# forestagostinelli/DeepCubeA

Hardware: AMD Instinct MI355X
Metric: A* nodes expanded/sec on cube3, batch 20k (higher is better)
Workload: dtype u8 states / f64 cost keys / f32 heuristic

## Files before the change

### deepcubea_amd/csrc/dca_engine.hip

```cpp
#include <string.h>

#include <new>
#include <vector>

#include "dca_common.h"
#include "dca_tile.h"

namespace dca {

constexpr int NBIN = 4096;
constexpr int kBinsPerThread = NBIN / 1024;
constexpr int kLgNbin = 12;
constexpr int kSub = 2048;
constexpr int kScanBlocks = 256;
constexpr int kCollectBlocks = 512;
constexpr int kRankBlocks = 256;
constexpr uint32_t kTinyBin = 512;
constexpr int kSortCap = 8192;
constexpr int RT = 512;
constexpr int kRegEnt = 16;
constexpr uint32_t kLdsEnt = RT * kRegEnt;
constexpr int kStash = 2560;
constexpr int kSegs = NBIN + 1 + kSub;
constexpr uint32_t kGiantBin = 8192;
// ... 119 lines not shown
    uint32_t* coop_off;
    uint64_t* part;
    uint64_t* tmp_key;
    uint32_t* tmp_id;
    uint16_t* tmp_f;
    uint32_t* tmp_idx;
    uint64_t* ord_key;
    uint32_t* ord_id;
    uint32_t* big_list;
    uint64_t* pop_key;
    uint32_t *pop_id, *pop_g;
    uint32_t *child_slot, *child_next, *child_v0;
    uint8_t *child_flags, *child_multi;
    float* child_h;
    uint8_t* nnet_in;
    uint8_t* onehot;
    uint8_t* root_nnet;
    int32_t* d_moves;
    Ctl* ctl;
    unsigned long long* prof;
    uint32_t* kept_pos;
    uint32_t* pk_n;
    uint32_t* pk_src;
    uint8_t* pk_nnet;
    uint8_t* pk_onehot;
    const float* pk_h;
    uint32_t pk_stride, inst;
    int pk_dtype;
};

__device__ __forceinline__ const IterState& st_cur(const Ctl* c) { return c->S[c->iters & 1]; }
__device__ __forceinline__ const IterState& st_next(const Ctl* c) { return c->S[(c->iters + 1) & 1]; }

__device__ __forceinline__ void fresh_binning(const Ctl* c, uint32_t buf, uint64_t& kmin, uint32_t& shift) {
    kmin = c->rng[buf].kmin;
    uint64_t kmax = c->rng[buf].kmax;
    const uint64_t T = c->T;
    if (T != ~0ull && T > kmax) kmax = T;
    shift = kmax > kmin ? select_shift(kmin, kmax) : 0u;
}

struct Stamp {
    unsigned long long* p;
    unsigned long long t0;
    __device__ __forceinline__ Stamp(const Eng& E, int kid) : p(nullptr), t0(0) {
        if (E.prof != nullptr && threadIdx.x == 0) {
            p = E.prof + ((size_t)kid * kProfSlots + (blockIdx.x & (kProfSlots - 1))) * 2;
            t0 = wall_clock64();
        }
    }
    __device__ __forceinline__ ~Stamp() {
        if (p) {
            atomicMin(p, t0);
            atomicMax(p + 1, (unsigned long long)wall_clock64());
        }
    }
};

__device__ __forceinline__ void prof_begin(const Eng& E, int kid) {
    if (E.prof != nullptr && threadIdx.x == 0)
        atomicMin(E.prof + ((size_t)kid * kProfSlots + (blockIdx.x & (kProfSlots - 1))) * 2, (unsigned long long)wall_clock64());
}
__device__ __forceinline__ void prof_end(const Eng& E, int kid) {
    if (E.prof != nullptr && threadIdx.x == 0)
        atomicMax(E.prof + ((size_t)kid * kProfSlots + (blockIdx.x & (kProfSlots - 1))) * 2 + 1, (unsigned long long)wall_clock64());
}

__device__ __forceinline__ void open_append(const Eng& E, Ctl* c, uint32_t buf, bool pred, uint64_t key, uint32_t id) {
    unsigned long long mask = __ballot(pred);
    if (mask == 0) return;
    int lane = threadIdx.x & 63;
    int leader = __ffsll((long long)mask) - 1;
    uint32_t cnt = (uint32_t)__popcll(mask);
    uint32_t basep = 0;
    uint64_t kmn = pred ? key : ~0ull, kmx = pred ? key : 0ull;
    for (int o = 32; o > 0; o >>= 1) {
        uint64_t a = __shfl_xor(kmn, o), b = __shfl_xor(kmx, o);
        kmn = a < kmn ? a : kmn;
        kmx = b > kmx ? b : kmx;
    }
    if (lane == leader) {
        basep = atomicAdd(&c->open_n[buf].v, cnt);
        atomicMin((unsigned long long*)&c->rng[buf].kmin, (unsigned long long)kmn);
        atomicMax((unsigned long long*)&c->rng[buf].kmax, (unsigned long long)kmx);
    }
    basep = __shfl(basep, leader);
    if (pred) {
        uint32_t pos = basep + (uint32_t)__popcll(mask & ((1ull << lane) - 1ull));
        if (pos < (buf < 2 ? E.front_cap : E.max_nodes)) {
            E.open_key[buf][pos] = key;
            E.open_id[buf][pos] = id;
        } else {
            c->failed = 1;
        }
    }
}
// ... 1022 lines not shown
                    const uint32_t p = atomicAdd(&L.st_n, 1u);
                    keys[idx] = DEAD;
                    if (p < (uint32_t)kStashG) {
                        st_key[p] = k[i];
                        st_idx[p] = idx;
                        st_f[p] = (uint16_t)f;
                        if (atomicAdd(&lcnt[f], 1u) == 0u) nzf[atomicAdd(&L.nz_n, 1u)] = (uint16_t)f;
                    } else {
                        const uint32_t pos = seg_base(f) + atomicAdd(&E.fill[f], 1u);
                        if (pos < seg_end(f)) {
                            E.tmp_key[pos] = k[i];
                            E.tmp_id[pos] = id[i];
                            E.tmp_f[pos] = (uint16_t)f;
                            E.tmp_idx[pos] = idx;
                        } else {
                            c->failed = 1;
                        }
                    }
                }
            }
            __syncthreads();
            if (L.st_n + TILE_D > (uint32_t)kStashG) flush();
        }
    }
    __syncthreads();
    flush();
    return BAR_PASS;
}

template <bool FUSED>
__global__ __launch_bounds__(256) void k_sel_collect(const Eng* __restrict__ engs) {
    const Eng& E = engs[blockIdx.y];
    Ctl* c = E.ctl;
    if (c->done) return;
    Stamp stamp(E, P_SEL_COLLECT);
    extern __shared__ __attribute__((aligned(16))) uint8_t collect_lds[];
    CollectLds& L = *reinterpret_cast<CollectLds*>(collect_lds);
    const uint32_t t = threadIdx.x;
    SelParams P;
    {
        const uint32_t b = c->cur_f, on0 = c->open_n[0].v, on1 = c->open_n[1].v;
        P.b = b;
        P.n = b ? on1 : on0;
        P.kmin = c->sel_kmin;
        P.shift = c->shift;
        P.want = c->want;
    }
    if constexpr (FUSED) {
        constexpr int PER = NBIN / 256;
        const uint32_t lane = t & 63, wv = t >> 6;
        uint32_t v[PER], sum = 0;
        {
            const uint4* h4 = reinterpret_cast<const uint4*>(E.hist + PER * t);
#pragma unroll
            for (int q = 0; q < PER / 4; q++) {
                const uint4 x = h4[q];
                v[4 * q] = x.x;
                v[4 * q + 1] = x.y;
                v[4 * q + 2] = x.z;
                v[4 * q + 3] = x.w;
            }
#pragma unroll
            for (int k = 0; k < PER; k++) sum += v[k];
        }
        uint32_t incl = sum;
        for (int o = 1; o < 64; o <<= 1) {
            const uint32_t u = __shfl_up(incl, o);
            if (lane >= (uint32_t)o) incl += u;
        }
        if (lane == 63) L.wsum[wv] = incl;
        if (t == 0) L.bstar = 0;
        __syncthreads();
        uint32_t run = incl - sum;
        for (uint32_t w = 0; w < wv; w++) run += L.wsum[w];
        const uint32_t want = P.want;
#pragma unroll
        for (int k = 0; k < PER; k++) {
            L.pre[PER * t + k] = run;
            if (run < want && want <= run + v[k]) L.bstar = PER * t + k;
            run += v[k];
        }
        if (t == 255) L.pre[NBIN] = run;
        __syncthreads();
        if (want == 0) {
            if (blockIdx.x == 0 && t == 0) {
                c->failed = 1;
                c->done = 1;
            }
            return;
// ... 134 lines not shown
                const uint32_t f = bin_of(k[i], kmin, shift);
                const uint32_t p = atomicAdd(&L.st_n, 1u);
                keys[idx] = DEAD;
                if (p < kStash) {
                    st_key[p] = k[i];
                    st_idx[p] = idx;
                    st_f[p] = (uint16_t)f;
                    if (atomicAdd(&L.lcnt[f], 1u) == 0u) nzf[atomicAdd(&L.nz_n, 1u)] = (uint16_t)f;
                } else {
                    const uint32_t pos = L.pre[f] + atomicAdd(&E.fill[f], 1u);
                    if (pos < L.pre[f + 1]) {
                        E.tmp_key[pos] = k[i];
                        E.tmp_id[pos] = ids[idx];
                        E.tmp_f[pos] = (uint16_t)f;
                        E.tmp_idx[pos] = idx;
                    } else {
                        c->failed = 1;
                    }
                }
            }
        }
        __syncthreads();
        if (L.st_n + TILE > (uint32_t)kStash) flush();
    }
    __syncthreads();
    flush();
}


constexpr int kRankStack = 512;
constexpr uint32_t kDirectMax = 512;
constexpr uint32_t kSubMax = 512;

struct RankItem {
    uint32_t off, n, need, src;
    uint32_t g, G;
    uint32_t nopush;
};
struct RankShared {
    uint32_t cnt[kSub + 64];
    uint32_t off[kSub + 1];
    uint32_t wsum[16];
    uint64_t red_lo[32], red_hi[32];
    uint64_t vmin_hi, vmin_lo;
    uint64_t kmin, kspan;
    uint32_t imin, ispan;
    uint32_t bits, tsub, sp, fail;
    uint32_t ret_base, ret_cnt;
    RankItem stack[kRankStack];
};

__device__ __forceinline__ void emit_pop(const Eng& E, Ctl* c, uint32_t rank, uint64_t key, uint32_t id) {
    E.pop_key[rank] = key;
    E.pop_id[rank] = id;
    if (id & ID_SOLVED) {
        if (E.sem == DCA_SEM_PY)
            atomicMin(&c->goal_best, ((unsigned long long)(uint32_t)E.g[id & ID_MASK] << 32) | rank);
        else
            atomicMin(&c->first_solved, rank);
    }
}
__device__ __forceinline__ void emit_ranked(const Eng& E, Ctl* c, uint32_t nf, bool live, uint32_t rank, uint32_t want,
                                            uint64_t key, uint32_t id) {
    if (live && rank < want) emit_pop(E, c, rank, key, id);
    const bool back = live && rank >= want;
    const unsigned long long mask = __ballot(back);
    if (mask == 0) return;
    const int lane = threadIdx.x & 63;
    const int leader = __ffsll((long long)mask) - 1;
    uint32_t basep = 0;
    if (lane == leader) basep = atomicAdd(&c->ret_n.v, (uint32_t)__popcll(mask));
    basep = __shfl(basep, leader);
    if (back) {
        const uint32_t slot = E.tmp_idx[basep + (uint32_t)__popcll(mask & ((1ull << lane) - 1ull))];
        E.open_key[nf][slot] = key;
        E.open_id[nf][slot] = id;
    }
}
__device__ __forceinline__ void ret_begin(Ctl* c, RankShared& S, uint32_t nf, uint32_t count) {
    __syncthreads();
    if (threadIdx.x == 0) {
        S.ret_base = count ? atomicAdd(&c->ret_n.v, count) : 0u;
        S.ret_cnt = 0;
    }
    __syncthreads();
}
struct RetAcc {};
__device__ __forceinline__ void ret_put(const Eng& E, Ctl* c, RankShared& S, uint32_t nf, bool pred, uint64_t key,
                                        uint32_t id, RetAcc& acc) {
    const unsigned long long mask = __ballot(pred);
    if (mask == 0) return;
    const int lane = threadIdx.x & 63;
    const int leader = __ffsll((long long)mask) - 1;
    uint32_t basep = 0;
    if (lane == leader) basep = atomicAdd(&S.ret_cnt, (uint32_t)__popcll(mask));
    basep = __shfl(basep, leader);
    if (pred) {
        const uint32_t slot = E.tmp_idx[S.ret_base + basep + (uint32_t)__popcll(mask & ((1ull << lane) - 1ull))];
        E.open_key[nf][slot] = key;
        E.open_id[nf][slot] = id;
    }
}
__device__ __forceinline__ void ret_end(Ctl* c, uint32_t nf, RetAcc acc) {}
template <int NJ>
__device__ __forceinline__ void ret_put_many(const Eng& E, RankShared& S, uint32_t nf, uint32_t n_ord, uint32_t preds,
                                             const uint64_t* key, const uint32_t* id) {
    const uint32_t cnt = (uint32_t)__popc(preds);
    const int lane = threadIdx.x & 63;
    uint32_t incl = cnt;
    for (int o = 1; o < 64; o <<= 1) {
        const uint32_t u = __shfl_up(incl, o);
        if (lane >= o) incl += u;
    }
    const uint32_t total = __shfl(incl, 63);
    if (total == 0) return;
    uint32_t basep = 0;
    if (lane == 63) basep = atomicAdd(&S.ret_cnt, total);
    basep = __shfl(basep, 63);
    uint32_t r = S.ret_base + basep + incl - cnt;
    uint32_t slot[NJ];
#pragma unroll
    for (int j = 0; j < NJ; j++) {
        slot[j] = E.tmp_idx[r < n_ord ? r : n_ord - 1];
        r += (preds >> j) & 1u;
    }
#pragma unroll
    for (int j = 0; j < NJ; j++)
        if ((preds >> j) & 1u) {
            E.open_key[nf][slot[j]] = key[j];
            E.open_id[nf][slot[j]] = id[j];
        }
}

__device__ __forceinline__ void rank_small_entries(const Eng& E, Ctl* c, RankShared& S, uint64_t* LK, uint32_t* LI,
                                                   uint32_t nf, uint32_t p0, uint32_t n_ord, uint32_t want) {
    const uint32_t t = threadIdx.x;
    const uint32_t plast = (p0 + RT - 1 < n_ord ? p0 + RT - 1 : n_ord - 1);
    const uint32_t f_lo = E.tmp_f[p0], f_hi = E.tmp_f[plast];
    const uint32_t lo = E.pre[f_lo], hi = E.pre[f_hi + 1];
    const bool staged = hi - lo <= kLdsEnt && f_hi - f_lo + 2 <= (uint32_t)kSub;
    if (staged) {
        for (uint32_t i = t; i < hi - lo; i += RT) {
            LK[i] = E.tmp_key[lo + i];
            LI[i] = E.tmp_id[lo + i];
        }
        for (uint32_t i = t; i < f_hi - f_lo + 2; i += RT) S.off[i] = E.pre[f_lo + i];
    }
    __syncthreads();
    const uint32_t p = p0 + t;
    bool live = p < n_ord;
    uint64_t k = 0;
    uint32_t id = 0, rank = 0;
    if (live) {
        const uint32_t f = E.tmp_f[p];
        const uint32_t o = staged ? S.off[f - f_lo] : E.pre[f], e = staged ? S.off[f - f_lo + 1] : E.pre[f + 1];
        if (e - o > kTinyBin) {
            live = false;
        } else if (staged) {
            k = LK[p - lo];
            id = LI[p - lo];
            rank = o;
            for (uint32_t j = o - lo; j < e - lo; j++) rank += pair_less(LK[j], LI[j], k, id) ? 1u : 0u;
        } else {
            k = E.tmp_key[p];
            id = E.tmp_id[p];
            rank = o;
            for (uint32_t j = o; j < e; j++) rank += pair_less(E.tmp_key[j], E.tmp_id[j], k, id) ? 1u : 0u;
        }
    }
    emit_ranked(E, c, nf, live, rank, want, k, id);
    __syncthreads();
// ... 88 lines not shown
    if (lane == 63) S.wsum[wv] = incl;
    __syncthreads();
    uint32_t run = incl - s4;
    for (uint32_t w = 0; w < wv; w++) run += S.wsum[w];
#pragma unroll
    for (int k = 0; k < PER; k++) {
        const uint32_t i = PER * t + k;
        if (i < nsub) {
            S.off[i] = run;
            S.cnt[i] = 0;
            if (run < need && need <= run + v[k]) S.tsub = i;
            if (i + 1 == nsub) S.off[nsub] = run + v[k];
        }
        run += v[k];
    }
    __syncthreads();
}

__device__ __forceinline__ void rank_push(RankShared& S, const RankItem& it, uint32_t tsub, uint32_t need, bool refinable,
                                          uint32_t lo = 0u, uint32_t hi = ~0u) {
    for (uint32_t sb = lo + threadIdx.x; sb <= tsub && sb < hi; sb += RT) {
        const uint32_t s0 = S.off[sb], e0 = S.off[sb + 1];
        if (e0 - s0 > kSubMax && refinable) {
            const uint32_t slot = atomicAdd(&S.sp, 1u);
            if (slot < (uint32_t)kRankStack)
                S.stack[slot] = RankItem{it.off + s0, e0 - s0, sb == tsub ? need - s0 : e0 - s0, it.src ^ 1u, 0u, 1u,
                                         (it.G > 1u || it.nopush) ? 1u : 0u};
            else
                S.fail = 1;
        }
    }
}

__device__ __noinline__ void rank_item(const Eng& E, Ctl* c, RankShared& S, uint64_t* LK, uint32_t* LI, uint32_t nf,
                                       uint32_t want, RankItem it) {
    const uint32_t t = threadIdx.x;
    const uint64_t* __restrict__ K = (it.src ? E.ord_key : E.tmp_key) + it.off;
    const uint32_t* __restrict__ I = (it.src ? E.ord_id : E.tmp_id) + it.off;
    uint64_t* __restrict__ K2 = (it.src ? E.tmp_key : E.ord_key) + it.off;
    uint32_t* __restrict__ I2 = (it.src ? E.tmp_id : E.ord_id) + it.off;
    const uint32_t n = it.n, need = it.need;
    if (n <= kDirectMax) {
        if (t < n) {
            LK[t] = K[t];
            LI[t] = I[t];
        }
        __syncthreads();
        ret_begin(c, S, nf, n - need);
        RetAcc acc{};
        const bool live = t < n;
        uint64_t k = 0;
        uint32_t id = 0, rank = 0;
        if (live) {
            k = LK[t];
            id = LI[t];
            for (uint32_t j = 0; j < n; j++) rank += pair_less(LK[j], LI[j], k, id) ? 1u : 0u;
            if (rank < need) emit_pop(E, c, it.off + rank, k, id);
        }
        ret_put(E, c, S, nf, live && rank >= need, k, id, acc);
        ret_end(c, nf, acc);
        __syncthreads();
        return;
    }
    uint32_t lg = 0;
    while ((8u << lg) <= n && lg < 11) lg++;
    if (lg < 11) lg++;
    if (n <= kLdsEnt) {
        uint64_t ek[kRegEnt];
// ... 18 lines not shown
            }
            rank_range64(S, kmn, kmx, imn, imx);
        }
        prof_end(E, P_RB_LOAD);
        prof_begin(E, P_RB_COUNT);
        const bool idmode = S.kspan == 0;
        const uint64_t kbase = S.kmin, span = idmode ? (uint64_t)S.ispan : S.kspan;
        const uint32_t ibase = S.imin;
        const uint32_t bits = span ? (uint32_t)(64 - __clzll((long long)span)) : 0u;
        if (lg > bits) lg = bits;
        const uint32_t nsub = 1u << lg, shc = bits - lg;
        const bool refinable = (shc > 0 || !idmode) && !it.nopush;
        const uint32_t lo_sub = (uint32_t)((uint64_t)nsub * it.g / it.G), hi_sub = (uint32_t)((uint64_t)nsub * (it.g + 1u) / it.G);
#pragma unroll
        for (int j = 0; j < kRegEnt; j++) {
            ek[j] = idmode ? (uint64_t)((ei[j] & ID_MASK) - ibase) : ek[j] - kbase;
            if (t + (uint32_t)RT * j < n) atomicAdd(&S.cnt[(uint32_t)(ek[j] >> shc)], 1u);
        }
        __syncthreads();
        rank_prefix(S, nsub, need);
        prof_end(E, P_RB_COUNT);
        prof_begin(E, P_RB_SCATTER);
        if (E.prof != nullptr) {
            uint32_t mx = 0;
            for (uint32_t sb = t; sb < nsub; sb += RT) mx = max(mx, S.off[sb + 1] - S.off[sb]);
            if (mx > 16) atomicMax(&c->dbg_maxsub, mx);
        }
        const uint32_t tsub = S.tsub;
        const bool tsub_pushed = S.off[tsub + 1] - S.off[tsub] > kSubMax && refinable;
        const uint32_t in_hi = hi_sub < tsub + 1u ? hi_sub : tsub + 1u;
        const uint32_t ret_lo = lo_sub > tsub + 1u ? lo_sub : tsub + 1u;
        ret_begin(c, S, nf, (ret_lo < hi_sub ? S.off[hi_sub] - S.off[ret_lo] : 0u) +
                                ((tsub >= lo_sub && tsub < hi_sub && !tsub_pushed) ? S.off[tsub + 1] - need : 0u));
        const uint32_t n_ord = c->n_ord;
        {
            uint32_t inm = 0, retm = 0, pos[kRegEnt];
#pragma unroll
            for (int j = 0; j < kRegEnt; j++) {
                const uint32_t sub = (uint32_t)(ek[j] >> shc);
                const bool live = t + (uint32_t)RT * j < n, in = live && sub >= lo_sub && sub < in_hi;
                inm |= (in ? 1u : 0u) << j;
                retm |= (live && sub >= ret_lo && sub < hi_sub ? 1u : 0u) << j;
                pos[j] = S.off[in ? sub : 0u] + atomicAdd(&S.cnt[in ? sub : (uint32_t)kSub + (t & 63u)], in ? 1u : 0u);
            }
#pragma unroll
            for (int j = 0; j < kRegEnt; j++) {
                if ((inm >> j) & 1u) {
                    LK[pos[j]] = ek[j];
                    LI[pos[j]] = ei[j];
                }
                ek[j] = idmode ? kbase : kbase + ek[j];
            }
            ret_put_many<kRegEnt>(E, S, nf, n_ord, retm, ek, ei);
        }
        __syncthreads();
        prof_end(E, P_RB_SCATTER);
        prof_begin(E, P_RB_ORDER);
        const uint32_t p_lo = S.off[lo_sub], p_hi = in_hi > lo_sub ? S.off[in_hi] : p_lo;
        constexpr int U = 4;
        for (uint32_t p0 = p_lo; p0 < p_hi; p0 += RT * U) {
            uint64_t o[U];
            uint32_t id[U], s0[U], cn[U], rank[U], livem = 0, bigm = 0, trip = 0;
#pragma unroll
            for (int u = 0; u < U; u++) {
                const uint32_t p = p0 + (uint32_t)u * RT + t;
                livem |= (p < p_hi ? 1u : 0u) << u;
                o[u] = LK[p < p_hi ? p : p_hi - 1];
// ... 54 lines not shown
#pragma unroll
            for (int j = 0; j < kRegEnt; j++)
                if (b0 + t + (uint32_t)RT * j < n) {
                    const u128 v = comp_of(ek[j], ei[j]);
                    vmin = v < vmin ? v : vmin;
                    vmax = v > vmax ? v : vmax;
                }
        }
        rank_range(S, vmin, vmax);
    }
    const u128 base = ((u128)S.vmin_hi << 64) | S.vmin_lo;
    const uint32_t bits = S.bits;
    if (lg > bits) lg = bits;
    const uint32_t nsub = 1u << lg, shc = bits - lg;
    for (uint32_t b0 = 0; b0 < n; b0 += kLdsEnt) {
        uint64_t ek[kRegEnt];
        uint32_t ei[kRegEnt];
#pragma unroll
        for (int j = 0; j < kRegEnt; j++) {
            const uint32_t i = b0 + t + (uint32_t)RT * j, ic = i < n ? i : n - 1;
            ek[j] = K[ic];
            ei[j] = I[ic];
        }
#pragma unroll
        for (int j = 0; j < kRegEnt; j++)
            if (b0 + t + (uint32_t)RT * j < n) atomicAdd(&S.cnt[sub_of(ek[j], ei[j], base, shc, nsub)], 1u);
    }
    __syncthreads();
    rank_prefix(S, nsub, need);
    const uint32_t tsub = S.tsub;
    const bool tsub_pushed = S.off[tsub + 1] - S.off[tsub] > kSubMax && shc > 0;
    ret_begin(c, S, nf, (n - S.off[tsub + 1]) + (tsub_pushed ? 0u : S.off[tsub + 1] - need));
    RetAcc acc{};
    const uint32_t n_ord_all = c->n_ord;
    for (uint32_t b0 = 0; b0 < n; b0 += kLdsEnt) {
        uint64_t ek[kRegEnt];
        uint32_t ei[kRegEnt];
#pragma unroll
        for (int j = 0; j < kRegEnt; j++) {
            const uint32_t i = b0 + t + (uint32_t)RT * j, ic = i < n ? i : n - 1;
            ek[j] = K[ic];
            ei[j] = I[ic];
        }
        uint32_t retm = 0;
#pragma unroll
        for (int j = 0; j < kRegEnt; j++) {
            const bool live = b0 + t + (uint32_t)RT * j < n;
            uint32_t sub = 0;
            if (live) {
                sub = sub_of(ek[j], ei[j], base, shc, nsub);
                if (sub <= tsub) {
                    const uint32_t p = S.off[sub] + atomicAdd(&S.cnt[sub], 1u);
                    K2[p] = ek[j];
                    I2[p] = ei[j];
                }
            }
            retm |= (live && sub > tsub ? 1u : 0u) << j;
        }
        ret_put_many<kRegEnt>(E, S, nf, n_ord_all, retm, ek, ei);
    }
    __syncthreads();
    const uint32_t m = S.off[tsub + 1];
    for (uint32_t p0 = 0; p0 < m; p0 += RT) {
        const uint32_t p = p0 + t;
        bool live = p < m;
        uint64_t k = 0;
        uint32_t id = 0, rank = 0;
        if (live) {
            k = K2[p];
            id = I2[p];
            const uint32_t sub = sub_of(k, id, base, shc, nsub);
            const uint32_t s0 = S.off[sub], e0 = S.off[sub + 1];
            if (e0 - s0 > kSubMax && shc > 0) {
                live = false;
            } else {
                rank = s0;
                for (uint32_t j = s0; j < e0; j++) rank += pair_less(K2[j], I2[j], k, id) ? 1u : 0u;
                if (rank < need) emit_pop(E, c, it.off + rank, k, id);
            }
        }
        ret_put(E, c, S, nf, live && rank >= need, k, id, acc);
    }
    rank_push(S, it, tsub, need, shc > 0);
    ret_end(c, nf, acc);
    __syncthreads();
}

__global__ __launch_bounds__(RT) void k_rank(const Eng* __restrict__ engs) {
    const Eng& E = engs[blockIdx.y];
    Ctl* c = E.ctl;
    if (c->done) return;
    Stamp stamp(E, P_RANK);
    __shared__ RankShared S;
    extern __shared__ __attribute__((aligned(16))) uint8_t rank_lds[];
    uint64_t* LK = reinterpret_cast<uint64_t*>(rank_lds);
    uint32_t* LI = reinterpret_cast<uint32_t*>(rank_lds + (size_t)kLdsEnt * 8);
    const uint32_t t = threadIdx.x;
    const uint32_t nf = c->cur_f;
    const uint32_t tseg = c->tseg, want = c->want;
    const uint32_t n_big = c->n_big, n_ord = c->n_ord;
    if (blockIdx.x == gridDim.x - 1) {
        const uint32_t bstar = c->bstar, pre_b = c->pre_b, cn_star = c->cn_star;
        if (want != 0) {
            for (uint32_t bin = t; bin < bstar; bin += RT) E.hist[bin] = 0;
            if (t == 0) E.hist[bstar] = cn_star - (want - pre_b);
        }
        for (uint32_t i = t; i < (uint32_t)kSegs; i += RT) E.fill[i] = 0;
        if (c->giant)
            for (uint32_t i = t; i < (uint32_t)(kMaxLevels * kSub); i += RT) E.subhist[i] = 0;
    }
    {
        Stamp sub(E, P_RANK_SMALL);
        for (uint32_t p0 = blockIdx.x * RT; p0 < n_ord; p0 += gridDim.x * RT)
            rank_small_entries(E, c, S, LK, LI, nf, p0, n_ord, want);
    }
    Stamp sub2(E, P_RANK_BIG);
    for (uint32_t bi = (blockIdx.x + gridDim.x - 64u) % gridDim.x; bi < n_big; bi += gridDim.x) {
        const uint32_t unit = E.big_list[bi];
        const uint32_t f = unit & 0xFFFFu;
        const uint32_t o = E.pre[f], n = E.pre[f + 1] - o;
        __syncthreads();
        if (t == 0) {
            S.stack[0] = RankItem{o, n, (f == tseg) ? want - o : n, 0u, (unit >> 16) & 15u, unit >> 20, 0u};
            S.sp = 1;
            S.fail = 0;
        }
        for (;;) {
            __syncthreads();
            const uint32_t sp = S.sp;
            if (sp == 0 || sp > (uint32_t)kRankStack) break;
            const RankItem it = S.stack[sp - 1];
            __syncthreads();
            if (t == 0) S.sp = sp - 1;
            __syncthreads();
            rank_item(E, c, S, LK, LI, nf, want, it);
        }
        if (t == 0 && (S.fail || S.sp != 0)) c->failed = 1;
    }
}

__device__ __forceinline__ void close_pop(const Eng& E, Ctl* c, const IterState& S0, uint32_t it, uint32_t want,
                                          uint32_t npop, uint32_t base, bool fail) {
    IterState N = S0;
    if (E.sem == DCA_SEM_PY) {
        const unsigned long long gb = c->goal_best;
        if (gb != ~0ull) {
            c->stop_after = 1;
            c->goal_id = E.pop_id[(uint32_t)(gb & 0xFFFFFFFFull)] & ID_MASK;
        }
    } else {
        const uint32_t fs = c->first_solved;
        if (fs != NIL) {
            const float cst = (float)cost_of_key(E.pop_key[fs]);
            if (E.B == 1) {
                N.best_id = E.pop_id[fs] & ID_MASK;
                N.best_cost = cst;
                N.has_best = 1;
                c->stop_after = 1;
            } else if (!S0.has_best || S0.best_cost > cst) {
                N.best_id = E.pop_id[fs] & ID_MASK;
                N.best_cost = cst;
                N.has_best = 1;
            }
        }
        if (S0.has_best && (float)cost_of_key(E.pop_key[0]) >= N.best_cost) c->stop_after = 1;
    }
    if (fail) {
        c->failed = 1;
        c->done = 1;
        c->front_dead.v -= want;
        return;
    }
    const uint32_t m = npop * (uint32_t)E.A;
    N.npop = npop;
    N.m = m;
    N.base = base;
    N.pool_n = base + m;
    c->S[(it + 1) & 1] = N;
    c->gen += (int64_t)m;
    c->expanded += npop;
}

constexpr uint8_t F_KEEP = 1, F_MIN = 2, F_NEW = 4;

// ... 20 lines not shown
            }
        }
    } else {
        uint32_t z = 0xFFFFu;
#pragma unroll
        for (int b = 3; b >= 0; b--)
            if (4 * w + b < (uint32_t)EV::D && ((pw >> (8 * b)) & 0xFFu) == 0u) z = 4 * w + b;
        for (int o = 8; o > 0; o >>= 1) {
            const uint32_t y = (uint32_t)__shfl_xor((int)z, o);
            z = y < z ? y : z;
        }
        z = z < (uint32_t)EV::D ? z : 0u;
        const uint32_t sw = (uint32_t)npuzzle_swap(DIM, (int)z, (int)a);
#pragma unroll
        for (uint32_t b = 0; b < 4; b++) {
            const uint32_t i = 4 * w + b;
            const uint32_t src = i < (uint32_t)EV::D ? ((i == z) ? sw : i) : 0u;
            const uint32_t v = (uint32_t)__shfl((int)pw, gbase + (int)(src >> 2));
            if (i < (uint32_t)EV::D) out |= ((i == sw) ? 0u : ((v >> (8 * (src & 3))) & 0xFFu)) << (8 * b);
        }
    }
    return out;
}

constexpr int kEngTile = 16;
template <int ENV, int DIM, int OH>
__global__ __launch_bounds__(kThreads) void k_expand(const Eng* __restrict__ engs, int heur_id, int write_nn) {
    const Eng& E = engs[blockIdx.y];
    using EV = EnvT<ENV, DIM>;
    using TL = Tile<ENV, DIM, kEngTile>;
    constexpr int kTileParents = kEngTile;
    constexpr int TP = kEngTile;
    Ctl* c = E.ctl;
    if (c->done) return;
    Stamp stamp(E, P_EXPAND);
    extern __shared__ __attribute__((aligned(16))) uint8_t smem[];
    uint8_t* lpar = smem;
    uint8_t* ltab = smem + TL::PAR_BYTES;
    uint8_t* lst = smem + TL::LDS_BYTES;
    __shared__ uint32_t l_pid[TP], l_g[TP];
    __shared__ uint32_t l_qn, l_qcc[kThreads], l_qrep[kThreads], l_qres[kThreads];
    __shared__ uint32_t l_ohq;
    static_assert((EV::D + 3) / 4 < 16, "no spare lane per row for the parent's path cost");
    const uint32_t it = (uint32_t)c->iters;
    const IterState S0 = c->S[it & 1];
    const uint32_t want = c->want;
    uint32_t npop = want;
    if (E.sem == DCA_SEM_CPP) {
        const uint32_t fs = c->first_solved;
        if (fs != NIL) npop = fs + 1;
    }
    const uint32_t base = (S0.pool_n + 15u) & ~15u;
    const bool fail = (uint64_t)base + (uint64_t)npop * (uint64_t)EV::A > (uint64_t)E.max_nodes;
    const uint32_t cur_new = c->cur_f;
    if (blockIdx.x == 0 && threadIdx.x == 0) close_pop(E, c, S0, it, want, npop, base, fail);
    if (fail) return;
    const uint32_t r0 = blockIdx.x * kTileParents;
    if (E.sem == DCA_SEM_CPP && r0 + kTileParents > npop) {
        uint32_t r = r0 + threadIdx.x;
        bool back = threadIdx.x < kTileParents && r >= npop && r < want;
        open_append(E, c, cur_new, back, back ? E.pop_key[r] : 0, back ? E.pop_id[r] : 0);
        if (back) atomicAdd(&E.hist[bin_of(E.pop_key[r], c->sel_kmin, c->shift)], 1u);
    }
    if (r0 >= npop) return;
    const uint32_t np = min((uint32_t)kTileParents, npop - r0);
    if (OH != 0 && threadIdx.x == 0) l_ohq = 0;
    {
        constexpr int WPR = (EV::D + 3) / 4;
        static_assert(WPR <= 16, "row wider than 64 bytes");
        const uint32_t w = threadIdx.x & 15;
#pragma unroll
        for (uint32_t r = threadIdx.x >> 4; r < (uint32_t)TP; r += 16) {
        if (r < np && w == WPR) {
            const uint32_t pid = E.pop_id[r0 + r] & ID_MASK;
            l_pid[r] = pid;
            l_g[r] = (uint32_t)E.g[pid];
        }
        if (r < np && w < WPR) {
            const uint8_t* row = E.state + (size_t)(E.pop_id[r0 + r] & ID_MASK) * EV::D;
            uint32_t v = 0;
            if (4 * w + 4 <= EV::D) {
                __builtin_memcpy(&v, row + 4 * w, 4);
            } else {
                for (int b = 0; 4 * w + b < EV::D; b++) v |= (uint32_t)row[4 * w + b] << (8 * b);
            }
#pragma unroll
            for (int b = 0; b < 4; b++)
                if (4 * w + b < EV::D) lpar[r * EV::D + 4 * w + b] = (uint8_t)(v >> (8 * b));
        }
        }
    }
    if constexpr (ENV == DCA_ENV_CUBE3) stage_tables<ENV, DIM>(ltab, lpar, np);
    __syncthreads();
    if constexpr (ENV != DCA_ENV_CUBE3) {
        stage_tables<ENV, DIM>(ltab, lpar, np);
        __syncthreads();
    }
    TL t{lpar, ltab};
    const uint32_t nchild = np * EV::A;
    const uint32_t j0 = r0 * EV::A;

    auto oh_emit = [&]() {
        if constexpr (OH != 0) {
            constexpr uint32_t ROW = EV::D * EV::DEPTH;
            constexpr uint32_t EPC = 16 / OH;
            const uint32_t te = nchild * ROW;
            const uint32_t one16 = E.oh_dtype == DCA_DT_F16 ? 0x3C00u : 0x3F80u;
            uint8_t* goh = E.onehot + (size_t)j0 * ROW * OH;
            const uint32_t nch = (te + EPC - 1) / EPC;
            auto staged_nnet = [&](uint32_t i) -> uint32_t {
                const uint32_t b = lst[i];
                return ENV == DCA_ENV_CUBE3 ? (b * 57u) >> 9 : b;
// ... 396 lines not shown
}

__device__ __forceinline__ void commit_ticket(const Eng& E, Ctl* c) {
    __syncthreads();
    if (threadIdx.x == 0) {
        uint32_t t = atomicAdd(&c->ticket_a.v, 1u);
        if (t == gridDim.x - 1) {
            c->ticket_a.v = 0;
            c->iters += 1;
            if (c->stop_after || c->failed) {
                c->done = 1;
            } else {
                const uint32_t fb = c->cur_f;
                const uint32_t live = __hip_atomic_load(&c->open_n[fb].v, __ATOMIC_RELAXED, __HIP_MEMORY_SCOPE_AGENT) -
                                      __hip_atomic_load(&c->front_dead.v, __ATOMIC_RELAXED, __HIP_MEMORY_SCOPE_AGENT) - c->front_above;
                c->want = live < (uint32_t)E.B ? live : (uint32_t)E.B;
                c->ret_n.v = 0;
                c->goal_best = ~0ull;
                c->first_solved = NIL;
                c->gbar.v = 0;
                c->grange.kmin = ~0ull;
                c->grange.kmax = 0;
                c->grange.imin = ~0u;
                c->grange.imax = 0;
            }
        }
    }
}

template <bool FUSED>
__global__ __launch_bounds__(1024) void k_commit(const Eng* __restrict__ engs, int packed) {
    const Eng& E = engs[blockIdx.y];
    Ctl* c = E.ctl;
    if (c->done) return;
    Stamp stamp(E, P_COMMIT);
    __shared__ uint32_t sh[3 * 16 + 3];
    __shared__ uint32_t lh[NBIN];
    __shared__ uint64_t red[4][16];
    const IterState& S1 = st_next(c);
    const uint32_t m = S1.m, base = S1.base;
    const uint32_t fb = c->cur_f, bb = c->cur_b;
    const uint64_t T = c->T;
    const uint32_t j = blockIdx.x * 1024 + threadIdx.x;
    if (blockIdx.x * 1024 >= m) {
        commit_ticket(E, c);
        return;
    }
    uint64_t rng_snap;
    {
        const uint32_t sl = threadIdx.x < 4 ? threadIdx.x : 0u;
        const uint32_t sbuf = sl < 2 ? fb : bb;
        const uint64_t* sp = (sl & 1) ? &c->rng[sbuf].kmax : &c->rng[sbuf].kmin;
        asm volatile("global_load_dwordx2 %0, %1, off" : "=v"(rng_snap) : "v"(sp) : "memory");
    }
    for (int k = 0; k < kBinsPerThread; k++) lh[kBinsPerThread * threadIdx.x + k] = 0;
    const uint64_t bin_kmin = c->sel_kmin;
    const uint32_t bin_shift = c->shift;
    __syncthreads();
    const bool live = j < m;
    const uint32_t id = base + j;
    bool keep = false, is_new = false;
    uint32_t gj = 0, my_slot = 0;
    float h_early = 0.f;
    uint8_t solved_early = 0;
    if (live) {
        if (!packed) h_early = E.child_h[j];
        solved_early = E.solved[id];
        const uint8_t fl = E.child_flags[j];
        is_new = (fl & F_NEW) != 0;
        gj = E.pop_g[j / (uint32_t)E.A] + 1u;
        const uint32_t slot = E.child_slot[j];
        my_slot = slot;
        bool is_min;
        uint32_t first = j;
        bool multi = false;
        if constexpr (FUSED) {
            multi = E.child_multi[j] != 0;
            const Dec d = decide_child(E, base, m, j, slot, E.child_v0[j], gj, multi);
            keep = d.keep;
            is_min = d.is_min;
            first = d.first;
        } else {
            keep = (fl & F_KEEP) != 0;
            is_min = (fl & F_MIN) != 0;
        }
        if (keep && is_min) {
            E.tab[slot].g = gj;
            if (E.sem == DCA_SEM_CPP) {
                uint32_t rep = (uint32_t)E.tab[slot].entry;
                if (FUSED && rep >= base) rep = base + first;
                if (rep != id) {
                    E.g[rep] = (int32_t)gj;
                    E.parent[rep] = E.parent[id];
                    E.move[rep] = E.move[id];
                }
            }
        }
        if (FUSED && multi && j == first) fix_representative(E, base, slot, id);
        E.child_multi[j] = 0;
    }
    uint64_t key = 0;
    uint32_t pid_flag = 0;
    if (keep) {
        const float hraw = packed ? E.pk_h[E.kept_pos[j]] : h_early;
        const float hv = fmaxf(hraw, 0.0f);
        const bool ns = solved_early == 0;
        pid_flag = ns ? 0u : ID_SOLVED;
        double cost;
        if (E.sem == DCA_SEM_PY) {
            cost = __dadd_rn(__dmul_rn(E.w, (double)gj), __dmul_rn((double)hv, ns ? 1.0 : 0.0));
        } else {
            cost = (double)__fadd_rn(__fmul_rn(hv, ns ? 1.0f : 0.0f), __fmul_rn(E.wf, (float)gj));
        }
        key = key_of_cost(cost);
    }
    const bool tof = keep && key <= T, tob = keep && key > T;
    const uint32_t hbin = c->hbin;
    if (tof) {
        const uint32_t f = bin_of(key, bin_kmin, bin_shift);
        if (f < hbin) atomicAdd(&lh[f], 1u);
    }
    const uint32_t cnt[3] = {tof ? 1u : 0u, tob ? 1u : 0u, is_new ? 1u : 0u};
    uint32_t* const ctr[3] = {&c->open_n[fb].v, &c->open_n[bb].v, &c->closed_n.v};
    uint32_t pos[3];
    block_reserveK<1024, 3>(cnt, ctr, pos, sh);
    static_assert(kBinsPerThread % 2 == 0, "bins are flushed in aligned pairs");
    if (kBinsPerThread * threadIdx.x < hbin) {
#pragma unroll
        for (int k = 0; k < kBinsPerThread; k += 2) {
            const uint32_t v0 = lh[kBinsPerThread * threadIdx.x + k], v1 = lh[kBinsPerThread * threadIdx.x + k + 1];
            if (v0 | v1)
                atomicAdd(reinterpret_cast<unsigned long long*>(&E.hist[kBinsPerThread * threadIdx.x + k]),
                          (unsigned long long)v0 | ((unsigned long long)v1 << 32));
        }
    }
    if (is_new && pos[2] < E.max_nodes) E.closed_slots[pos[2]] = my_slot;
    if (tof) {
        if (pos[0] < E.front_cap) {
            E.open_key[fb][pos[0]] = key;
            E.open_id[fb][pos[0]] = id | pid_flag;
        } else {
            c->failed = 1;
        }
    } else if (tob) {
        if (pos[1] < E.max_nodes) {
            E.open_key[bb][pos[1]] = key;
            E.open_id[bb][pos[1]] = id | pid_flag;
        } else {
            c->failed = 1;
        }
// ... 1019 lines not shown
```

Before: 94.75 million.

## Hoist control and input loads to kernel heads across collect, rank, expand, commit

Across several kernels, the control-block fields, histogram slices, per-child inputs and per-parent pop ids are now loaded in one batch at kernel entry, before the done check. Empty asm statements force these loads to be issued early so their latencies overlap instead of being serialised behind dependent branches. The rank kernel also gets a compact RankEng struct whose pointers are pinned to scalar registers through a constant-address-space load and readfirstlane. The cost is speculative loads, using clamped indices, on blocks that would otherwise exit early, plus higher register pressure.

Result: no change. 95.18 million, median of 4 (+0.5%).

```diff
diff --git a/deepcubea_amd/csrc/dca_engine.hip b/deepcubea_amd/csrc/dca_engine.hip
--- a/deepcubea_amd/csrc/dca_engine.hip
+++ b/deepcubea_amd/csrc/dca_engine.hip
@@ -175,6 +175,19 @@
 __device__ __forceinline__ const IterState& st_cur(const Ctl* c) { return c->S[c->iters & 1]; }
 __device__ __forceinline__ const IterState& st_next(const Ctl* c) { return c->S[(c->iters + 1) & 1]; }
 
+using GCtl = const __attribute__((address_space(1))) Ctl*;
+__device__ __forceinline__ GCtl global_ctl(const Ctl* c) { return (GCtl)c; }
+__device__ __forceinline__ IterState load_state(GCtl c, int k) {
+    IterState s;
+    s.pool_n = c->S[k].pool_n;
+    s.npop = c->S[k].npop;
+    s.m = c->S[k].m;
+    s.base = c->S[k].base;
+    s.best_id = c->S[k].best_id;
+    s.has_best = c->S[k].has_best;
+    s.best_cost = c->S[k].best_cost;
+    return s;
+}
 __device__ __forceinline__ void fresh_binning(const Ctl* c, uint32_t buf, uint64_t& kmin, uint32_t& shift) {
     kmin = c->rng[buf].kmin;
     uint64_t kmax = c->rng[buf].kmax;
@@ -186,7 +199,8 @@
 struct Stamp {
     unsigned long long* p;
     unsigned long long t0;
-    __device__ __forceinline__ Stamp(const Eng& E, int kid) : p(nullptr), t0(0) {
+    template <class EngT>
+    __device__ __forceinline__ Stamp(const EngT& E, int kid) : p(nullptr), t0(0) {
         if (E.prof != nullptr && threadIdx.x == 0) {
             p = E.prof + ((size_t)kid * kProfSlots + (blockIdx.x & (kProfSlots - 1))) * 2;
             t0 = wall_clock64();
@@ -200,11 +214,13 @@
     }
 };
 
-__device__ __forceinline__ void prof_begin(const Eng& E, int kid) {
+template <class EngT>
+__device__ __forceinline__ void prof_begin(const EngT& E, int kid) {
     if (E.prof != nullptr && threadIdx.x == 0)
         atomicMin(E.prof + ((size_t)kid * kProfSlots + (blockIdx.x & (kProfSlots - 1))) * 2, (unsigned long long)wall_clock64());
 }
-__device__ __forceinline__ void prof_end(const Eng& E, int kid) {
+template <class EngT>
+__device__ __forceinline__ void prof_end(const EngT& E, int kid) {
     if (E.prof != nullptr && threadIdx.x == 0)
         atomicMax(E.prof + ((size_t)kid * kProfSlots + (blockIdx.x & (kProfSlots - 1))) * 2 + 1, (unsigned long long)wall_clock64());
 }
@@ -1293,29 +1309,42 @@
 __global__ __launch_bounds__(256) void k_sel_collect(const Eng* __restrict__ engs) {
     const Eng& E = engs[blockIdx.y];
     Ctl* c = E.ctl;
-    if (c->done) return;
+    const GCtl gc = global_ctl(c);
+    const uint32_t t = threadIdx.x;
+    constexpr int PER = NBIN / 256;
+    const int32_t done = gc->done;
+    const uint32_t hb = gc->cur_f, on0 = gc->open_n[0].v, on1 = gc->open_n[1].v;
+    const uint64_t hkmin = gc->sel_kmin;
+    const uint32_t hshift = gc->shift, hwant = gc->want;
+    typedef uint32_t u32x4 __attribute__((ext_vector_type(4)));
+    u32x4 hx[PER / 4] = {};
+    if constexpr (FUSED) {
+        const u32x4* h4 = reinterpret_cast<const u32x4*>(E.hist + PER * t);
+#pragma unroll
+        for (int q = 0; q < PER / 4; q++) hx[q] = h4[q];
+        asm volatile("" ::"v"(done), "v"(hb), "v"(on0), "v"(on1), "v"(hkmin), "v"(hshift), "v"(hwant), "v"(hx[0]), "v"(hx[1]),
+                     "v"(hx[2]), "v"(hx[3]));
+    } else {
+        asm volatile("" ::"v"(done), "v"(hb), "v"(on0), "v"(on1), "v"(hkmin), "v"(hshift), "v"(hwant));
+    }
+    if (done) return;
     Stamp stamp(E, P_SEL_COLLECT);
     extern __shared__ __attribute__((aligned(16))) uint8_t collect_lds[];
     CollectLds& L = *reinterpret_cast<CollectLds*>(collect_lds);
-    const uint32_t t = threadIdx.x;
     SelParams P;
-    {
-        const uint32_t b = c->cur_f, on0 = c->open_n[0].v, on1 = c->open_n[1].v;
-        P.b = b;
-        P.n = b ? on1 : on0;
-        P.kmin = c->sel_kmin;
-        P.shift = c->shift;
-        P.want = c->want;
-    }
+    P.b = hb;
+    P.n = hb ? on1 : on0;
+    P.kmin = hkmin;
+    P.shift = hshift;
+    P.want = hwant;
     if constexpr (FUSED) {
-        constexpr int PER = NBIN / 256;
+        static_assert(PER == 16, "the head requests four 16-byte pieces of the histogram per thread");
         const uint32_t lane = t & 63, wv = t >> 6;
         uint32_t v[PER], sum = 0;
         {
-            const uint4* h4 = reinterpret_cast<const uint4*>(E.hist + PER * t);
 #pragma unroll
             for (int q = 0; q < PER / 4; q++) {
-                const uint4 x = h4[q];
+                const u32x4 x = hx[q];
                 v[4 * q] = x.x;
                 v[4 * q + 1] = x.y;
                 v[4 * q + 2] = x.z;
@@ -1516,6 +1545,59 @@
 constexpr uint32_t kDirectMax = 512;
 constexpr uint32_t kSubMax = 512;
 
+using CEng = const __attribute__((address_space(4))) Eng*;
+struct RankEng {
+    int sem;
+    uint32_t max_nodes;
+    unsigned long long* prof;
+    Ctl* ctl;
+    int32_t* g;
+    uint32_t *hist, *fill, *subhist, *big_list, *pre;
+    uint64_t *tmp_key, *ord_key, *pop_key;
+    uint32_t *tmp_id, *ord_id, *tmp_idx, *pop_id;
+    uint16_t* tmp_f;
+    uint64_t *fkey0, *fkey1;
+    uint32_t *fid0, *fid1;
+    __device__ __forceinline__ uint64_t* front_key(uint32_t nf) const { return nf ? fkey1 : fkey0; }
+    __device__ __forceinline__ uint32_t* front_id(uint32_t nf) const { return nf ? fid1 : fid0; }
+};
+__device__ __forceinline__ RankEng load_rank_eng(CEng e) {
+    {
+        const uint64_t a = (uint64_t)e;
+        const uint32_t lo = (uint32_t)__builtin_amdgcn_readfirstlane((int)(uint32_t)a);
+        const uint32_t hi = (uint32_t)__builtin_amdgcn_readfirstlane((int)(uint32_t)(a >> 32));
+        e = (CEng)(((uint64_t)hi << 32) | lo);
+    }
+    RankEng R;
+    R.sem = e->sem;
+    R.max_nodes = e->max_nodes;
+    R.prof = e->prof;
+    R.ctl = e->ctl;
+    R.g = e->g;
+    R.hist = e->hist;
+    R.fill = e->fill;
+    R.subhist = e->subhist;
+    R.big_list = e->big_list;
+    R.pre = e->pre;
+    R.tmp_key = e->tmp_key;
+    R.ord_key = e->ord_key;
+    R.pop_key = e->pop_key;
+    R.tmp_id = e->tmp_id;
+    R.ord_id = e->ord_id;
+    R.tmp_idx = e->tmp_idx;
+    R.pop_id = e->pop_id;
+    R.tmp_f = e->tmp_f;
+    R.fkey0 = e->open_key[0];
+    R.fkey1 = e->open_key[1];
+    R.fid0 = e->open_id[0];
+    R.fid1 = e->open_id[1];
+    asm volatile("" : "+s"(R.prof), "+s"(R.g), "+s"(R.big_list), "+s"(R.pre), "+s"(R.tmp_key), "+s"(R.ord_key), "+s"(R.pop_key),
+                 "+s"(R.tmp_id), "+s"(R.ord_id), "+s"(R.tmp_idx), "+s"(R.pop_id), "+s"(R.tmp_f));
+    asm volatile("" : "+s"(R.fkey0), "+s"(R.fkey1), "+s"(R.fid0), "+s"(R.fid1), "+s"(R.hist), "+s"(R.fill), "+s"(R.subhist),
+                 "+s"(R.sem), "+s"(R.max_nodes));
+    return R;
+}
+
 struct RankItem {
     uint32_t off, n, need, src;
     uint32_t g, G;
@@ -1534,7 +1616,7 @@
     RankItem stack[kRankStack];
 };
 
-__device__ __forceinline__ void emit_pop(const Eng& E, Ctl* c, uint32_t rank, uint64_t key, uint32_t id) {
+__device__ __forceinline__ void emit_pop(const RankEng& E, Ctl* c, uint32_t rank, uint64_t key, uint32_t id) {
     E.pop_key[rank] = key;
     E.pop_id[rank] = id;
     if (id & ID_SOLVED) {
@@ -1544,7 +1626,7 @@
             atomicMin(&c->first_solved, rank);
     }
 }
-__device__ __forceinline__ void emit_ranked(const Eng& E, Ctl* c, uint32_t nf, bool live, uint32_t rank, uint32_t want,
+__device__ __forceinline__ void emit_ranked(const RankEng& E, Ctl* c, uint32_t nf, bool live, uint32_t rank, uint32_t want,
                                             uint64_t key, uint32_t id) {
     if (live && rank < want) emit_pop(E, c, rank, key, id);
     const bool back = live && rank >= want;
@@ -1557,8 +1639,8 @@
     basep = __shfl(basep, leader);
     if (back) {
         const uint32_t slot = E.tmp_idx[basep + (uint32_t)__popcll(mask & ((1ull << lane) - 1ull))];
-        E.open_key[nf][slot] = key;
-        E.open_id[nf][slot] = id;
+        E.front_key(nf)[slot] = key;
+        E.front_id(nf)[slot] = id;
     }
 }
 __device__ __forceinline__ void ret_begin(Ctl* c, RankShared& S, uint32_t nf, uint32_t count) {
@@ -1570,7 +1652,7 @@
     __syncthreads();
 }
 struct RetAcc {};
-__device__ __forceinline__ void ret_put(const Eng& E, Ctl* c, RankShared& S, uint32_t nf, bool pred, uint64_t key,
+__device__ __forceinline__ void ret_put(const RankEng& E, Ctl* c, RankShared& S, uint32_t nf, bool pred, uint64_t key,
                                         uint32_t id, RetAcc& acc) {
     const unsigned long long mask = __ballot(pred);
     if (mask == 0) return;
@@ -1581,13 +1663,13 @@
     basep = __shfl(basep, leader);
     if (pred) {
         const uint32_t slot = E.tmp_idx[S.ret_base + basep + (uint32_t)__popcll(mask & ((1ull << lane) - 1ull))];
-        E.open_key[nf][slot] = key;
-        E.open_id[nf][slot] = id;
+        E.front_key(nf)[slot] = key;
+        E.front_id(nf)[slot] = id;
     }
 }
 __device__ __forceinline__ void ret_end(Ctl* c, uint32_t nf, RetAcc acc) {}
 template <int NJ>
-__device__ __forceinline__ void ret_put_many(const Eng& E, RankShared& S, uint32_t nf, uint32_t n_ord, uint32_t preds,
+__device__ __forceinline__ void ret_put_many(const RankEng& E, RankShared& S, uint32_t nf, uint32_t n_ord, uint32_t preds,
                                              const uint64_t* key, const uint32_t* id) {
     const uint32_t cnt = (uint32_t)__popc(preds);
     const int lane = threadIdx.x & 63;
@@ -1611,16 +1693,15 @@
 #pragma unroll
     for (int j = 0; j < NJ; j++)
         if ((preds >> j) & 1u) {
-            E.open_key[nf][slot[j]] = key[j];
-            E.open_id[nf][slot[j]] = id[j];
-        }
-}
-
-__device__ __forceinline__ void rank_small_entries(const Eng& E, Ctl* c, RankShared& S, uint64_t* LK, uint32_t* LI,
-                                                   uint32_t nf, uint32_t p0, uint32_t n_ord, uint32_t want) {
+            E.front_key(nf)[slot[j]] = key[j];
+            E.front_id(nf)[slot[j]] = id[j];
+        }
+}
+
+__device__ __forceinline__ void rank_small_entries(const RankEng& E, Ctl* c, RankShared& S, uint64_t* LK, uint32_t* LI,
+                                                   uint32_t nf, uint32_t p0, uint32_t n_ord, uint32_t want, uint32_t f_lo,
+                                                   uint32_t f_hi) {
     const uint32_t t = threadIdx.x;
-    const uint32_t plast = (p0 + RT - 1 < n_ord ? p0 + RT - 1 : n_ord - 1);
-    const uint32_t f_lo = E.tmp_f[p0], f_hi = E.tmp_f[plast];
     const uint32_t lo = E.pre[f_lo], hi = E.pre[f_hi + 1];
     const bool staged = hi - lo <= kLdsEnt && f_hi - f_lo + 2 <= (uint32_t)kSub;
     if (staged) {
@@ -1775,8 +1856,9 @@
     }
 }
 
-__device__ __noinline__ void rank_item(const Eng& E, Ctl* c, RankShared& S, uint64_t* LK, uint32_t* LI, uint32_t nf,
-                                       uint32_t want, RankItem it) {
+__device__ __noinline__ void rank_item(CEng ce, Ctl* c, RankShared& S, uint64_t* LK, uint32_t* LI, uint32_t nf,
+                                       uint32_t want, uint32_t n_ord, RankItem it) {
+    const RankEng E = load_rank_eng(ce);
     const uint32_t t = threadIdx.x;
     const uint64_t* __restrict__ K = (it.src ? E.ord_key : E.tmp_key) + it.off;
     const uint32_t* __restrict__ I = (it.src ? E.ord_id : E.tmp_id) + it.off;
@@ -1861,7 +1943,6 @@
         const uint32_t ret_lo = lo_sub > tsub + 1u ? lo_sub : tsub + 1u;
         ret_begin(c, S, nf, (ret_lo < hi_sub ? S.off[hi_sub] - S.off[ret_lo] : 0u) +
                                 ((tsub >= lo_sub && tsub < hi_sub && !tsub_pushed) ? S.off[tsub + 1] - need : 0u));
-        const uint32_t n_ord = c->n_ord;
         {
             uint32_t inm = 0, retm = 0, pos[kRegEnt];
 #pragma unroll
@@ -1982,7 +2063,6 @@
     const bool tsub_pushed = S.off[tsub + 1] - S.off[tsub] > kSubMax && shc > 0;
     ret_begin(c, S, nf, (n - S.off[tsub + 1]) + (tsub_pushed ? 0u : S.off[tsub + 1] - need));
     RetAcc acc{};
-    const uint32_t n_ord_all = c->n_ord;
     for (uint32_t b0 = 0; b0 < n; b0 += kLdsEnt) {
         uint64_t ek[kRegEnt];
         uint32_t ei[kRegEnt];
@@ -2007,7 +2087,7 @@
             }
             retm |= (live && sub > tsub ? 1u : 0u) << j;
         }
-        ret_put_many<kRegEnt>(E, S, nf, n_ord_all, retm, ek, ei);
+        ret_put_many<kRegEnt>(E, S, nf, n_ord, retm, ek, ei);
     }
     __syncthreads();
     const uint32_t m = S.off[tsub + 1];
@@ -2037,32 +2117,43 @@
 }
 
 __global__ __launch_bounds__(RT) void k_rank(const Eng* __restrict__ engs) {
-    const Eng& E = engs[blockIdx.y];
+    const CEng ce = (CEng)(engs + blockIdx.y);
+    const RankEng E = load_rank_eng(ce);
     Ctl* c = E.ctl;
-    if (c->done) return;
+    const GCtl gc = global_ctl(c);
+    const uint32_t t = threadIdx.x;
+    const int32_t done = gc->done;
+    const uint32_t nf = gc->cur_f;
+    const uint32_t tseg = gc->tseg, want = gc->want;
+    const uint32_t n_big = gc->n_big, n_ord = gc->n_ord;
+    const uint32_t bstar = gc->bstar, pre_b = gc->pre_b, cn_star = gc->cn_star, giant = gc->giant;
+    const uint32_t q0 = blockIdx.x * RT;
+    const uint32_t f_first = E.tmp_f[min(q0, E.max_nodes - 1u)], f_last = E.tmp_f[min(q0 + RT - 1u, E.max_nodes - 1u)];
+    asm volatile("" ::"v"(done), "v"(nf), "v"(tseg), "v"(want), "v"(n_big), "v"(n_ord), "v"(bstar), "v"(pre_b), "v"(cn_star),
+                 "v"(giant), "v"(f_first), "v"(f_last));
+    if (done) return;
     Stamp stamp(E, P_RANK);
     __shared__ RankShared S;
     extern __shared__ __attribute__((aligned(16))) uint8_t rank_lds[];
     uint64_t* LK = reinterpret_cast<uint64_t*>(rank_lds);
     uint32_t* LI = reinterpret_cast<uint32_t*>(rank_lds + (size_t)kLdsEnt * 8);
-    const uint32_t t = threadIdx.x;
-    const uint32_t nf = c->cur_f;
-    const uint32_t tseg = c->tseg, want = c->want;
-    const uint32_t n_big = c->n_big, n_ord = c->n_ord;
     if (blockIdx.x == gridDim.x - 1) {
-        const uint32_t bstar = c->bstar, pre_b = c->pre_b, cn_star = c->cn_star;
         if (want != 0) {
             for (uint32_t bin = t; bin < bstar; bin += RT) E.hist[bin] = 0;
             if (t == 0) E.hist[bstar] = cn_star - (want - pre_b);
         }
         for (uint32_t i = t; i < (uint32_t)kSegs; i += RT) E.fill[i] = 0;
-        if (c->giant)
+        if (giant)
             for (uint32_t i = t; i < (uint32_t)(kMaxLevels * kSub); i += RT) E.subhist[i] = 0;
     }
     {
         Stamp sub(E, P_RANK_SMALL);
-        for (uint32_t p0 = blockIdx.x * RT; p0 < n_ord; p0 += gridDim.x * RT)
-            rank_small_entries(E, c, S, LK, LI, nf, p0, n_ord, want);
+        for (uint32_t p0 = q0; p0 < n_ord; p0 += gridDim.x * RT) {
+            const bool whole = p0 + RT - 1 < n_ord;
+            const uint32_t f_lo = p0 == q0 ? f_first : (uint32_t)E.tmp_f[p0];
+            const uint32_t f_hi = (p0 == q0 && whole) ? f_last : (uint32_t)E.tmp_f[whole ? p0 + RT - 1 : n_ord - 1];
+            rank_small_entries(E, c, S, LK, LI, nf, p0, n_ord, want, f_lo, f_hi);
+        }
     }
     Stamp sub2(E, P_RANK_BIG);
     for (uint32_t bi = (blockIdx.x + gridDim.x - 64u) % gridDim.x; bi < n_big; bi += gridDim.x) {
@@ -2083,13 +2174,13 @@
             __syncthreads();
             if (t == 0) S.sp = sp - 1;
             __syncthreads();
-            rank_item(E, c, S, LK, LI, nf, want, it);
+            rank_item(ce, c, S, LK, LI, nf, want, n_ord, it);
         }
         if (t == 0 && (S.fail || S.sp != 0)) c->failed = 1;
     }
 }
 
-__device__ __forceinline__ void close_pop(const Eng& E, Ctl* c, const IterState& S0, uint32_t it, uint32_t want,
+__device__ __forceinline__ void close_pop(const Eng& E, Ctl* c, const IterState& S0, uint32_t fs, uint32_t it, uint32_t want,
                                           uint32_t npop, uint32_t base, bool fail) {
     IterState N = S0;
     if (E.sem == DCA_SEM_PY) {
@@ -2099,7 +2190,6 @@
             c->goal_id = E.pop_id[(uint32_t)(gb & 0xFFFFFFFFull)] & ID_MASK;
         }
     } else {
-        const uint32_t fs = c->first_solved;
         if (fs != NIL) {
             const float cst = (float)cost_of_key(E.pop_key[fs]);
             if (E.B == 1) {
@@ -2186,7 +2276,23 @@
     constexpr int kTileParents = kEngTile;
     constexpr int TP = kEngTile;
     Ctl* c = E.ctl;
-    if (c->done) return;
+    const GCtl gc = global_ctl(c);
+    static_assert(kThreads == 16 * TP, "one round of the row gather: 16 lanes per parent");
+    const uint32_t r0 = blockIdx.x * kTileParents;
+    const uint32_t* const p_pop = E.pop_id;
+    const uint32_t Bc = (uint32_t)E.B;
+    asm volatile("" ::"s"(gc), "s"(p_pop), "s"(Bc));
+    const int32_t done = gc->done;
+    const uint32_t it = (uint32_t)gc->iters;
+    const IterState Sa = load_state(gc, 0), Sb = load_state(gc, 1);
+    const uint32_t want = gc->want, cur_new = gc->cur_f, fs = gc->first_solved, sel_shift = gc->shift;
+    const uint64_t sel_kmin = gc->sel_kmin;
+    const uint32_t my_r = threadIdx.x >> 4;
+    const uint32_t my_pop = p_pop[min(r0 + my_r, Bc - 1u)];
+    asm volatile("" ::"v"(done), "v"(it), "v"(want), "v"(cur_new), "v"(fs), "v"(sel_shift), "v"(sel_kmin), "v"(my_pop), "v"(Sa.pool_n),
+                 "v"(Sa.best_id), "v"(Sa.has_best), "v"(Sa.best_cost), "v"(Sb.pool_n), "v"(Sb.best_id), "v"(Sb.has_best),
+                 "v"(Sb.best_cost));
+    if (done) return;
     Stamp stamp(E, P_EXPAND);
     extern __shared__ __attribute__((aligned(16))) uint8_t smem[];
     uint8_t* lpar = smem;
@@ -2196,25 +2302,20 @@
     __shared__ uint32_t l_qn, l_qcc[kThreads], l_qrep[kThreads], l_qres[kThreads];
     __shared__ uint32_t l_ohq;
     static_assert((EV::D + 3) / 4 < 16, "no spare lane per row for the parent's path cost");
-    const uint32_t it = (uint32_t)c->iters;
-    const IterState S0 = c->S[it & 1];
-    const uint32_t want = c->want;
+    const IterState S0 = (it & 1) ? Sb : Sa;
     uint32_t npop = want;
     if (E.sem == DCA_SEM_CPP) {
-        const uint32_t fs = c->first_solved;
         if (fs != NIL) npop = fs + 1;
     }
     const uint32_t base = (S0.pool_n + 15u) & ~15u;
     const bool fail = (uint64_t)base + (uint64_t)npop * (uint64_t)EV::A > (uint64_t)E.max_nodes;
-    const uint32_t cur_new = c->cur_f;
-    if (blockIdx.x == 0 && threadIdx.x == 0) close_pop(E, c, S0, it, want, npop, base, fail);
+    if (blockIdx.x == 0 && threadIdx.x == 0) close_pop(E, c, S0, fs, it, want, npop, base, fail);
     if (fail) return;
-    const uint32_t r0 = blockIdx.x * kTileParents;
     if (E.sem == DCA_SEM_CPP && r0 + kTileParents > npop) {
         uint32_t r = r0 + threadIdx.x;
         bool back = threadIdx.x < kTileParents && r >= npop && r < want;
         open_append(E, c, cur_new, back, back ? E.pop_key[r] : 0, back ? E.pop_id[r] : 0);
-        if (back) atomicAdd(&E.hist[bin_of(E.pop_key[r], c->sel_kmin, c->shift)], 1u);
+        if (back) atomicAdd(&E.hist[bin_of(E.pop_key[r], sel_kmin, sel_shift)], 1u);
     }
     if (r0 >= npop) return;
     const uint32_t np = min((uint32_t)kTileParents, npop - r0);
@@ -2223,15 +2324,15 @@
         constexpr int WPR = (EV::D + 3) / 4;
         static_assert(WPR <= 16, "row wider than 64 bytes");
         const uint32_t w = threadIdx.x & 15;
-#pragma unroll
-        for (uint32_t r = threadIdx.x >> 4; r < (uint32_t)TP; r += 16) {
+        {
+        const uint32_t r = my_r;
         if (r < np && w == WPR) {
-            const uint32_t pid = E.pop_id[r0 + r] & ID_MASK;
+            const uint32_t pid = my_pop & ID_MASK;
             l_pid[r] = pid;
             l_g[r] = (uint32_t)E.g[pid];
         }
         if (r < np && w < WPR) {
-            const uint8_t* row = E.state + (size_t)(E.pop_id[r0 + r] & ID_MASK) * EV::D;
+            const uint8_t* row = E.state + (size_t)(my_pop & ID_MASK) * EV::D;
             uint32_t v = 0;
             if (4 * w + 4 <= EV::D) {
                 __builtin_memcpy(&v, row + 4 * w, 4);
@@ -2694,16 +2795,35 @@
 __global__ __launch_bounds__(1024) void k_commit(const Eng* __restrict__ engs, int packed) {
     const Eng& E = engs[blockIdx.y];
     Ctl* c = E.ctl;
-    if (c->done) return;
+    const GCtl gc = global_ctl(c);
+    const uint32_t j = blockIdx.x * 1024 + threadIdx.x;
+    const float* const p_h = E.child_h;
+    const uint8_t *const p_flags = E.child_flags, *const p_multi = E.child_multi;
+    const uint32_t *const p_slot = E.child_slot, *const p_v0 = E.child_v0;
+    const uint32_t Mc = E.M;
+    asm volatile("" ::"s"(gc), "s"(p_h), "s"(p_flags), "s"(p_multi), "s"(p_slot), "s"(p_v0), "s"(Mc));
+    const uint32_t jc = min(j, Mc - 1u);
+    const float h_spec = packed ? 0.f : p_h[jc];
+    const uint8_t fl_spec = p_flags[jc];
+    const uint32_t slot_spec = p_slot[jc];
+    uint32_t multi_spec = 0, v0_spec = 0;
+    if constexpr (FUSED) {
+        multi_spec = p_multi[jc];
+        v0_spec = p_v0[jc];
+    }
+    const int32_t done = gc->done;
+    const uint32_t it = (uint32_t)gc->iters;
+    const uint32_t m_a = gc->S[0].m, base_a = gc->S[0].base, m_b = gc->S[1].m, base_b = gc->S[1].base;
+    const uint32_t fb = gc->cur_f, bb = gc->cur_b, hbin = gc->hbin, bin_shift = gc->shift;
+    const uint64_t T = gc->T, bin_kmin = gc->sel_kmin;
+    asm volatile("" ::"v"(done), "v"(it), "v"(m_a), "v"(base_a), "v"(m_b), "v"(base_b), "v"(fb), "v"(bb), "v"(hbin), "v"(bin_shift),
+                 "v"(T), "v"(bin_kmin), "v"(h_spec), "v"((uint32_t)fl_spec), "v"(slot_spec), "v"(multi_spec), "v"(v0_spec));
+    if (done) return;
     Stamp stamp(E, P_COMMIT);
     __shared__ uint32_t sh[3 * 16 + 3];
     __shared__ uint32_t lh[NBIN];
     __shared__ uint64_t red[4][16];
-    const IterState& S1 = st_next(c);
-    const uint32_t m = S1.m, base = S1.base;
-    const uint32_t fb = c->cur_f, bb = c->cur_b;
-    const uint64_t T = c->T;
-    const uint32_t j = blockIdx.x * 1024 + threadIdx.x;
+    const uint32_t m = (it & 1) ? m_a : m_b, base = (it & 1) ? base_a : base_b;
     if (blockIdx.x * 1024 >= m) {
         commit_ticket(E, c);
         return;
@@ -2716,8 +2836,6 @@
         asm volatile("global_load_dwordx2 %0, %1, off" : "=v"(rng_snap) : "v"(sp) : "memory");
     }
     for (int k = 0; k < kBinsPerThread; k++) lh[kBinsPerThread * threadIdx.x + k] = 0;
-    const uint64_t bin_kmin = c->sel_kmin;
-    const uint32_t bin_shift = c->shift;
     __syncthreads();
     const bool live = j < m;
     const uint32_t id = base + j;
@@ -2726,19 +2844,19 @@
     float h_early = 0.f;
     uint8_t solved_early = 0;
     if (live) {
-        if (!packed) h_early = E.child_h[j];
+        h_early = h_spec;
         solved_early = E.solved[id];
-        const uint8_t fl = E.child_flags[j];
+        const uint8_t fl = fl_spec;
         is_new = (fl & F_NEW) != 0;
         gj = E.pop_g[j / (uint32_t)E.A] + 1u;
-        const uint32_t slot = E.child_slot[j];
+        const uint32_t slot = slot_spec;
         my_slot = slot;
         bool is_min;
         uint32_t first = j;
         bool multi = false;
         if constexpr (FUSED) {
-            multi = E.child_multi[j] != 0;
-            const Dec d = decide_child(E, base, m, j, slot, E.child_v0[j], gj, multi);
+            multi = multi_spec != 0;
+            const Dec d = decide_child(E, base, m, j, slot, v0_spec, gj, multi);
             keep = d.keep;
             is_min = d.is_min;
             first = d.first;
@@ -2777,7 +2895,6 @@
         key = key_of_cost(cost);
     }
     const bool tof = keep && key <= T, tob = keep && key > T;
-    const uint32_t hbin = c->hbin;
     if (tof) {
         const uint32_t f = bin_of(key, bin_kmin, bin_shift);
         if (f < hbin) atomicAdd(&lh[f], 1u);
```
